# bacpop/sparrowhawk

Hardware: AMD Instinct MI355X
Metric: Gbases/s assembled, k=31 150bp reads (higher is better)
Workload: dtype u64

## Files before the change

sparrowhawk_amd/csrc/count_part.h:

```cpp
#pragma once
#include <hip/hip_runtime.h>
#include <stdint.h>
#include <type_traits>
#include "kmer.h"

namespace shk {

static constexpr int PART_THREADS = 1024;
static constexpr int COUNT_THREADS = 1024;
static constexpr int PART_MAX_P = 16384;

struct PartParams {
    uint32_t P, G, slice_cap;
    int k, m;
    uint32_t max_n;
};

template <int RW> struct Rec { uint64_t w[RW]; };

__device__ __forceinline__ uint64_t sel4(uint32_t b, uint64_t t0, uint64_t t1, uint64_t t2, uint64_t t3) {
    uint64_t lo = (b & 1) ? t1 : t0;
    uint64_t hi = (b & 1) ? t3 : t2;
    return (b & 2) ? hi : lo;
}
// ... 586 lines not shown
    const unsigned long long gbase = ((unsigned long long)ctl.emit_base_hi << 32) | ctl.emit_base_lo;
    for (uint32_t i = threadIdx.x; i < n_emit; i += COUNT_THREADS) {
        const uint32_t sl = list[i];
        const unsigned long long o = gbase + i;
        if (o < out_cap) {
            Kmer<W> x;
            if constexpr (W == 1) x.w[0] = tb.key0[sl];
            else {
#pragma unroll
                for (int j = 0; j < W; j++) x.w[j] = tb.key[j][sl];
            }
            out_keys.store(o, x);
            out_cnt[o] = tb.cnt[sl];
        }
    }
}

struct OvfRec { uint32_t p, est_distinct; unsigned long long instances; };
struct OvfItem { uint32_t p, F, cap, pad; unsigned long long base; };
static constexpr uint32_t OVF_MAX_F = 256;

struct RunView {
    const unsigned long long *run_addr16;
    const uint32_t *run_cnt;
    uint32_t S;
    int k;
    const uint32_t *weights = nullptr;
    unsigned long long rec_base16 = 0;
};

__global__ __launch_bounds__(256) void k_make_runs(const uint32_t *__restrict__ fill, PartParams pp,
                                                   const uint64_t *recs, uint32_t rec_words,
                                                   unsigned long long *__restrict__ run_addr16,
                                                   uint32_t *__restrict__ run_cnt) {
    const uint64_t n = (uint64_t)pp.P * pp.G;
    const unsigned long long base16 = (unsigned long long)recs >> 4;
    for (uint64_t i = (uint64_t)blockIdx.x * blockDim.x + threadIdx.x; i < n; i += (uint64_t)gridDim.x * blockDim.x) {
        run_addr16[i] = base16 + i * pp.slice_cap * (rec_words / 2u);
        run_cnt[i] = min(fill[i], pp.slice_cap);
    }
}

__global__ __launch_bounds__(256) void k_part_totals(const uint32_t *__restrict__ fill, PartParams pp,
                                                     unsigned long long *__restrict__ totals) {
    const uint32_t p = blockIdx.x;
    unsigned long long t = 0;
    for (uint32_t g = threadIdx.x; g < pp.G; g += blockDim.x) t += min(fill[(uint64_t)p * pp.G + g], pp.slice_cap);
    for (int o = 32; o > 0; o >>= 1) t += __shfl_down(t, o);
    __shared__ unsigned long long part[4];
    if ((threadIdx.x & 63) == 0) part[threadIdx.x >> 6] = t;
    __syncthreads();
    if (threadIdx.x == 0) totals[p] = part[0] + part[1] + part[2] + part[3];
}

template <int RW>
__global__ __launch_bounds__(256) void k_pack_partition(const uint64_t *__restrict__ recs,
                                                        const uint32_t *__restrict__ fill, PartParams pp,
                                                        const unsigned long long *__restrict__ base,
                                                        uint64_t *__restrict__ dst) {
    __shared__ uint32_t pre[257];
    const uint32_t p = blockIdx.x;
    const int lane = threadIdx.x & 63;
    if (threadIdx.x < 64) {
        uint32_t run = 0;
        for (uint32_t g0 = 0; g0 < pp.G; g0 += 64) {
            const uint32_t g = g0 + threadIdx.x;
            const uint32_t f = g < pp.G ? min(fill[(uint64_t)p * pp.G + g], pp.slice_cap) : 0u;
            uint32_t incl = f;
            for (int o = 1; o < 64; o <<= 1) { uint32_t v = __shfl_up(incl, o); if (lane >= o) incl += v; }
            if (g < pp.G) pre[g] = run + incl - f;
            run += __shfl(incl, 63);
        }
        if (threadIdx.x == 0) pre[pp.G] = run;
// ... 912 lines not shown
```

sparrowhawk_amd/csrc/pipeline.hip:

```cpp
#include <hip/hip_runtime.h>
#include <hipcub/hipcub.hpp>
#include <thread>
#include <stdint.h>
#include <stdio.h>
#include <stdlib.h>
#include <string.h>
#include <algorithm>
#include <atomic>
#include <chrono>
#include <map>
#include <memory>
#include <mutex>
#include <string>
#include <vector>

#include "kmer.h"
#include "pipeline.h"
#include "shard_comm.h"
#include "unitig_graph.h"

namespace shk {

#define HIPCHK(call)                                                                      \
    do {                                                                                  \
// ... 300 lines not shown
}

static constexpr uint32_t ARRIVAL_SLAB = 64u << 10;
__global__ __launch_bounds__(256) void k_text_to_host(const char *__restrict__ src, char *__restrict__ dst_host, unsigned long long bytes,
                                                      uint32_t n_slabs, uint32_t *__restrict__ flags_host) {
    for (uint32_t s = blockIdx.x; s < n_slabs; s += gridDim.x) {
        const unsigned long long o = (unsigned long long)s * ARRIVAL_SLAB;
        const uint32_t m = (uint32_t)(bytes - o < ARRIVAL_SLAB ? bytes - o : ARRIVAL_SLAB);
        const uint4 *a = reinterpret_cast<const uint4 *>(src + o);
        uint4 *d = reinterpret_cast<uint4 *>(dst_host + o);
        const uint32_t nv = m >> 4;
#pragma unroll 4
        for (uint32_t i = threadIdx.x; i < nv; i += 256) d[i] = a[i];
        if (threadIdx.x < (m & 15u)) dst_host[o + (nv << 4) + threadIdx.x] = src[o + (nv << 4) + threadIdx.x];
        __threadfence_system();
        __syncthreads();
        if (threadIdx.x == 0) __hip_atomic_store(&flags_host[s], 1u, __ATOMIC_RELEASE, __HIP_MEMORY_SCOPE_SYSTEM);
    }
}
__global__ __launch_bounds__(1024) void k_ends_to_host(const char *__restrict__ text, const unsigned long long *__restrict__ src ,
                                                       uint32_t nc, uint32_t E, char *__restrict__ ends_host, uint32_t *__restrict__ flag_host) {
    const unsigned long long total = (unsigned long long)nc * 2ull * E;
    for (unsigned long long t = threadIdx.x; t < total; t += blockDim.x) {
        const uint32_t c = (uint32_t)(t / (2ull * E)), r = (uint32_t)(t % (2ull * E)), side = r / E, j = r % E;
        const unsigned long long off = src[2 * c], len = src[2 * c + 1];
        const unsigned long long m = len < E ? len : (unsigned long long)E;
        char ch = 0;
        if (j < m) ch = side ? text[off + len - m + j] : text[off + j];
        ends_host[t] = ch;
    }
    __threadfence_system();
    __syncthreads();
    if (threadIdx.x == 0) __hip_atomic_store(flag_host, 1u, __ATOMIC_RELEASE, __HIP_MEMORY_SCOPE_SYSTEM);
}
__global__ __launch_bounds__(256) void k_text_to_host_planned(const char *__restrict__ src, char *__restrict__ dst_host,
                                                              const unsigned long long *__restrict__ plan) {
    if (plan[0] != 1ull) return;
    const unsigned long long bytes = plan[1];
    const unsigned long long nv = bytes >> 4;
    const uint4 *a = reinterpret_cast<const uint4 *>(src);
    uint4 *d = reinterpret_cast<uint4 *>(dst_host);
    for (unsigned long long i = (unsigned long long)blockIdx.x * 256u + threadIdx.x; i < nv; i += (unsigned long long)gridDim.x * 256u) d[i] = a[i];
    if (blockIdx.x == 0 && threadIdx.x < (bytes & 15ull)) dst_host[(nv << 4) + threadIdx.x] = src[(nv << 4) + threadIdx.x];
}
class SlabArrival : public TextArrival {
public:
    void set(char *dst, size_t bytes, volatile uint32_t *flags, uint32_t n_slabs, hipStream_t st) { base_ = dst; total_ = bytes; flags_ = flags; n_slabs_ = n_slabs; st_ = st; failed_.store(false); }
    const char *base() const override { return base_; }
    size_t total() const override { return total_; }
    static bool spin_until(volatile uint32_t *f, std::atomic<bool> &failed) {
        if (__atomic_load_n(f, __ATOMIC_ACQUIRE)) return true;
        const auto t0 = std::chrono::steady_clock::now();
        for (uint32_t it = 0;; it++) {
            if (__atomic_load_n(f, __ATOMIC_ACQUIRE)) return true;
            if (failed.load(std::memory_order_relaxed)) return false;
            if ((it & 0xFFFu) == 0xFFFu && std::chrono::steady_clock::now() - t0 > std::chrono::seconds(20)) { failed.store(true); return false; }
            __builtin_ia32_pause();
        }
    }
    void wait_range(size_t begin, size_t end) override {
        if (end > total_) end = total_;
        if (begin >= end) return;
        for (size_t s = begin / ARRIVAL_SLAB; s <= (end - 1) / ARRIVAL_SLAB; s++) if (!spin_until(flags_ + s, failed_)) return;
    }
    int finish(std::string &err) override {
        const hipError_t e = hipStreamSynchronize(st_);
        if (e != hipSuccess || failed_.load()) { err = std::string("download of the contigs failed") + (e != hipSuccess ? std::string(": ") + hipGetErrorString(e) : std::string()); return -5; }
        return 0;
    }
    std::atomic<bool> failed_{false};
private:
    char *base_ = nullptr; size_t total_ = 0; volatile uint32_t *flags_ = nullptr; uint32_t n_slabs_ = 0; hipStream_t st_ = nullptr;
};

static inline int part_win(int k) {
    static const int forced = [] { const char *e = getenv("SHK_PART_WIN"); return e ? atoi(e) : 0; }();
// ... 163 lines not shown
            if (env_u64("SHK_SLICE_NOSKEW", 0) == 0)
                while ((cap * RW * 8) % 2048 < 256 || (cap * RW * 8) % 2048 > 1792) cap++;
            if (cap * pp_.G > 0xFFFFFFF0ull) { err = "a partition would hold more than 2^32 records"; return -1; }
            pp_.slice_cap = (uint32_t)cap;
            const uint64_t n_slices = (uint64_t)P * pp_.G;
            if (int rc = recs_.alloc(n_slices * cap * RW, err)) return rc;
            if (int rc = fill_.alloc(n_slices, err)) return rc;
            HIPCHK(fill2_async(fill_.p, n_slices * 4, 0u, ctl_.p, CTL_WORDS * sizeof(unsigned long long), 0u, stream_));
            EvTimer t(stream_);
            if (h_bases && attempt == 0) {
                uint64_t C = env_u64("SHK_H2D_PIECES", 4);
                if (C < 1) C = 1;
                while (C > 1 && n_seg / C < (uint64_t)PART_THREADS * pp_.G) C--;
                if (!copy_stream_) copy_stream_ = stream_pool_get(stream_dev_ + 1000);
                if (!copy_stream_) HIPCHK(hipStreamCreateWithFlags(&copy_stream_, hipStreamNonBlocking));
                const uint64_t n_words = (n_bases + 15) / 16 + 1;
                std::vector<hipEvent_t> evs((size_t)C, nullptr);
                struct EvGuard { std::vector<hipEvent_t> &v; ~EvGuard() { for (auto e : v) if (e) (void)hipEventDestroy(e); } } evg{evs};
                struct CopyDrain { hipStream_t s; std::unique_lock<std::mutex> token; ~CopyDrain() { (void)hipStreamSynchronize(s); } }
                    copy_drain{copy_stream_, std::unique_lock<std::mutex>(upload_token(stream_dev_))};
                for (uint64_t c = 0; c < C; c++) {
                    const uint64_t s0 = n_seg * c / C, s1 = n_seg * (c + 1) / C;
                    const uint64_t w0 = h_seg_off[s0] >> 4, w1 = std::min<uint64_t>(n_words, (((uint64_t)h_seg_off[s1] + 15) >> 4) + 1);
                    HIPCHK(hipMemcpyAsync((void *)(d_seg_off + s0), h_seg_off + s0, (s1 - s0 + 1) * 4, hipMemcpyHostToDevice, copy_stream_));
                    HIPCHK(hipMemcpyAsync((void *)(d_bases + w0), h_bases + w0, (w1 - w0) * 4, hipMemcpyHostToDevice, copy_stream_));
                    HIPCHK(hipEventCreateWithFlags(&evs[c], hipEventDisableTiming));
                    HIPCHK(hipEventRecord(evs[c], copy_stream_));
                    HIPCHK(hipStreamWaitEvent(stream_, evs[c], 0));
                    launch_partition(wblk, d_bases, d_seg_off + s0, (uint32_t)(s1 - s0));
                }
                HIPCHK(hipGetLastError());
                times_.add("h2d_pieces_x1", (double)C);
                if (defer_p1_ && batches_.empty()) {
                    HIPCHK(hipMemcpyAsync(mbox64() + MB_P1, ctl_.p + 8, 16, hipMemcpyDeviceToHost, stream_));
                    t.stop_later("partition_with_upload", pending_timers_);
                    p1_ = P1Pending{true, d_bases, d_seg_off, n_seg, n_bases, cap};
                    return finish_partition(n_slices, err);
                }
                t.mark();
                unsigned long long h[2];
                HIPCHK(hipMemcpyAsync(h, ctl_.p + 8, sizeof h, hipMemcpyDeviceToHost, stream_));
                WAIT_STREAM();
                const uint32_t *fl = (const uint32_t *)&h[0];
                if (fl[1]) { err = "a read segment exceeds 32768 bases (split it on the host)"; return -1; }
                if ((uint32_t)h[1] <= cap) {
                    times_.add("partition_with_upload", t.elapsed());
                    if (int rc = finish_partition(n_slices, err)) return rc;
                    return 0;
                }
                times_.add("partition_retry", t.elapsed());
                cap = (uint64_t)(uint32_t)h[1] + 8;
                continue;
            }
            launch_partition_all(wblk, d_bases, d_seg_off, n_seg);
            HIPCHK(hipGetLastError());
            if (defer_p1_ && attempt == 0 && batches_.empty() && piece_list_.empty()) {
                HIPCHK(hipMemcpyAsync(mbox64() + MB_P1, ctl_.p + 8, 16, hipMemcpyDeviceToHost, stream_));
                t.stop_later("partition_kernel", pending_timers_);
                p1_ = P1Pending{true, d_bases, d_seg_off, n_seg, n_bases, cap};
                return finish_partition(n_slices, err);
            }
            t.mark();
            unsigned long long h[2];
            HIPCHK(hipMemcpyAsync(h, ctl_.p + 8, sizeof h, hipMemcpyDeviceToHost, stream_));
            WAIT_STREAM();
            const double ms = t.elapsed();
            const uint32_t *fl = (const uint32_t *)&h[0];
            if (fl[1]) { err = "a read segment exceeds 32768 bases (split it on the host)"; return -1; }
            const uint32_t max_fill = (uint32_t)h[1];
            if (max_fill <= cap) {
                times_.add("partition_kernel", ms);
                if (int rc = finish_partition(n_slices, err)) return rc;
                return 0;
            }
            times_.add("partition_retry", ms);
            cap = (uint64_t)max_fill + 8;
        }
        err = "partition slices overflowed twice";
        return -6;
    }

    int finish_partition(uint64_t n_slices, std::string &err) {
        constexpr int RW = 2 * W;
        have_parts_ = true;
        if (int rc = run_off_.alloc(n_slices, err)) return rc;
        if (int rc = run_cnt_.alloc(n_slices, err)) return rc;
        hipLaunchKernelGGL(k_make_runs, dim3(grid_for(n_slices)), dim3(256), 0, stream_, fill_.p, pp_, recs_.p,
                           (uint32_t)RW, run_off_.p, run_cnt_.p);
        HIPCHK(hipGetLastError());
        run_view_.run_addr16 = run_off_.p; run_view_.run_cnt = run_cnt_.p;
        run_view_.S = pp_.G; run_view_.k = k_; n_count_parts_ = pp_.P;
        return 0;
    }

    struct BatchRecs { DevBuf<uint64_t> dense; std::vector<unsigned long long> part_off;  };

    int pack_current_batch(std::string &err) {
        constexpr int RW = 2 * W;
        DevBuf<unsigned long long> tot, base;
        if (int rc = tot.alloc(pp_.P, err)) return rc;
        if (int rc = base.alloc(pp_.P, err)) return rc;
        hipLaunchKernelGGL(k_part_totals, dim3(pp_.P), dim3(256), 0, stream_, fill_.p, pp_, tot.p);
        HIPCHK(hipGetLastError());
        std::vector<unsigned long long> h(pp_.P);
        HIPCHK(hipMemcpyAsync(h.data(), tot.p, (size_t)pp_.P * 8, hipMemcpyDeviceToHost, stream_));
        WAIT_STREAM();
        std::unique_ptr<BatchRecs> b(new BatchRecs());
        b->part_off.assign(pp_.P + 1, 0);
        for (uint32_t p = 0; p < pp_.P; p++) b->part_off[p + 1] = b->part_off[p] + h[p];
        if (int rc = b->dense.alloc(b->part_off[pp_.P] * RW + 2, err)) return rc;
        HIPCHK(hipMemcpyAsync(base.p, b->part_off.data(), (size_t)pp_.P * 8, hipMemcpyHostToDevice, stream_));
        EvTimer t(stream_, stage_timers_);
        hipLaunchKernelGGL((k_pack_partition<2 * W>), dim3(pp_.P), dim3(256), 0, stream_, recs_.p, fill_.p, pp_, base.p, b->dense.p);
        HIPCHK(hipGetLastError());
        if (t.on()) times_.add("batch_pack_kernel", t.stop());
        WAIT_STREAM();
        batches_.push_back(std::move(b));
        recs_.release(); fill_.release(); run_off_.release(); run_cnt_.release(); have_parts_ = false;
        if (batches_.size() >= env_u64("SHK_MERGE_BATCHES_AT", 192)) return merge_batches(err);
        return 0;
    }

    int merge_batches(std::string &err) {
        constexpr int RW = 2 * W;
        if (batches_.size() < 2) return 0;
        if (int rc = make_batch_run_view(err)) return rc;
        std::unique_ptr<BatchRecs> m(new BatchRecs());
        m->part_off.assign(pp_.P + 1, 0);
        for (uint32_t p = 0; p < pp_.P; p++) {
            unsigned long long tot = 0;
            for (auto &b : batches_) tot += b->part_off[p + 1] - b->part_off[p];
// ... 23 lines not shown
            unsigned long long r = 0;
            for (uint32_t b = 0; b < nb; b++) r += batches_[b]->part_off[p + 1] - batches_[b]->part_off[p];
            if (r > 0xFFFFFFF0ull) { err = "a partition holds more than 2^32 records"; return -1; }
        }
        for (uint32_t p = 0; p < pp_.P; p++)
            for (uint32_t b = 0; b < nb; b++) {
                const BatchRecs &B = *batches_[b];
                const unsigned long long c = B.part_off[p + 1] - B.part_off[p];
                if (c > 0xFFFFFFFFull) { err = "partition too large in one batch"; return -1; }
                addr16[(uint64_t)p * nb + b] = ((unsigned long long)(uintptr_t)B.dense.p >> 4) + B.part_off[p] * (unsigned long long)W;
                cnt[(uint64_t)p * nb + b] = (uint32_t)c;
            }
        if (int rc = run_off_.alloc(n_runs, err)) return rc;
        if (int rc = run_cnt_.alloc(n_runs, err)) return rc;
        HIPCHK(hipMemcpyAsync(run_off_.p, addr16.data(), n_runs * 8, hipMemcpyHostToDevice, stream_));
        HIPCHK(hipMemcpyAsync(run_cnt_.p, cnt.data(), n_runs * 4, hipMemcpyHostToDevice, stream_));
        WAIT_STREAM();
        run_view_.run_addr16 = run_off_.p; run_view_.run_cnt = run_cnt_.p;
        run_view_.S = nb; run_view_.k = k_; n_count_parts_ = pp_.P;
        have_parts_ = true;
        return 0;
    }
    void set_bloom(bool on) override { bloom_ = on; }
    void set_verbose(bool on) override { if (on) { stage_timers_ = true; keep_stages_ = true; } }
    void single_batch_resident(bool on) override { defer_p1_ = on && !global_mode_; }
    void expect_more_batches() override { if (!forced_P_ && batches_.empty() && !have_parts_) forced_P_ = (uint32_t)PART_MAX_P; }

    int run_count_partitions(const RunView &rv, uint32_t n_parts, uint32_t threshold, DevBuf<uint64_t> (&keys)[W],
                             DevBuf<uint32_t> &cnt, uint64_t &n_rows, uint64_t hist_out[500], uint64_t &inst_out,
                             uint64_t cap_hint, double &ms_out, std::string &err) {
        if (n_parts == 0) { n_rows = 0; inst_out = 0; memset(hist_out, 0, 500 * 8); ms_out = 0; return 0; }
        constexpr uint32_t S = CountShared<W>::S;
        const bool repartition = env_u64("SHK_NO_REPARTITION", 0) == 0 && rv.weights == nullptr;
        DevBuf<unsigned long long> dh;
        DevBuf<OvfRec> d_ovf; DevBuf<OvfItem> d_items; DevBuf<uint32_t> d_fill, d_list, d_maxfill, d_new; DevBuf<uint64_t> d_kmers; DevBuf<BucketRef> d_blist; DevBuf<unsigned long long> d_sumfill;
        const bool bloom = bloom_ && !bloom_off_once_;
        unsigned long long bloom_new = 0, bloom_kmer_bytes = 0, bloom_kmer_bytes_exact = 0;
        if (int rc = dh.alloc(500, err)) return rc;
        if (repartition) if (int rc = d_ovf.alloc(n_parts, err)) return rc;
        const bool split = W <= 2 && repartition && !bloom && rv.weights == nullptr && split_ready_ && split_base_.size() == n_parts && split_total_ > 0 &&
                           env_u64("SHK_COUNT_SPLIT", 1) != 0;
        struct DropSplit { Pipeline<W> *me; bool on; ~DropSplit() { if (on) me->shard_drop_dedup(); } } drop_split{this, split};
        uint64_t cap = cap_hint;
        for (int attempt = 0; attempt < (bloom ? 4 : 2); attempt++) {
            bloom_new = 0; bloom_kmer_bytes = 0; bloom_kmer_bytes_exact = 0;
            for (int j = 0; j < W; j++) if (int rc = keys[j].alloc(cap, err)) return rc;
            if (int rc = cnt.alloc(cap, err)) return rc;
            HIPCHK(fill2_async(dh.p, 500 * 8, 0u, ctl_.p, CTL_WORDS * sizeof(unsigned long long), 0u, stream_));
            KeyArr<W> ok; for (int j = 0; j < W; j++) ok.w[j] = keys[j].p;
            const uint32_t probe_parts = (uint32_t)env_u64("SHK_PROBE_PARTS", 512);
            const uint32_t n_probe = (repartition && probe_parts && n_parts / 4 >= probe_parts) ? probe_parts : 0u;
            EvTimer t(stream_);
            if (split) {
                if (int rc = dd_base_.alloc(n_parts, err)) return rc;
                if (int rc = dd_n_.alloc(n_parts, err)) return rc;
                if (int rc = dd_recs_.alloc(split_total_ * 2 * W + 2, err)) return rc;
                if (int rc = dd_w_.alloc(split_total_ + 2, err)) return rc;
                if (split_stride_) {
                    hipLaunchKernelGGL(k_stride_fill, dim3((n_parts + 255) / 256), dim3(256), 0, stream_, dd_base_.p, n_parts, split_stride_);
                    HIPCHK(hipGetLastError());
                } else HIPCHK(hipMemcpyAsync(dd_base_.p, split_base_.data(), (size_t)n_parts * 8, hipMemcpyHostToDevice, stream_));
                const uint32_t defer_after = n_probe / 8;
                EvTimer t_a(stream_, stage_timers_);
                hipLaunchKernelGGL(k_dedupe_partitions<W>, dim3(std::min<uint32_t>(n_parts, 2u * (uint32_t)n_cus_)), dim3(COUNT_THREADS), 0, stream_,
                                   rv, 0u, n_parts, dd_base_.p, dd_recs_.p, dd_w_.p, dd_n_.p, (uint32_t *)(ctl_.p + 12),
                                   d_ovf.p, (uint32_t *)(ctl_.p + 3), defer_after, (S / 10) * 9, (uint32_t *)(ctl_.p + 14) + 1);
                HIPCHK(hipGetLastError());
                if (attempt == 0) t_a.stop_later("count_dedupe_kernel", pending_timers_);
                const uint32_t per_cu = 2u;
                uint32_t merge = (uint32_t)std::min<uint64_t>(std::max<uint64_t>(env_u64("SHK_COUNT_MERGE", 1), 1), 4);
                if (merge == 3) merge = 2;
                while (merge > 1 && (n_parts % merge != 0 || (n_parts / merge) % 256u != 0 || n_parts / merge < 2u * per_cu * (uint32_t)n_cus_)) merge >>= 1;
                const uint32_t n_groups = (n_parts + merge - 1) / merge;
                EmitRanges er{};
                er_groups_ = 0;
                if (n_parts % merge == 0 && (n_groups & (n_groups - 1u)) == 0 && n_groups <= GP_MAX && cap < (1ull << 28) &&
                    env_u64("SHK_GRAPH_RANGES", 1) != 0) {
                    if (int rc = er_off_.alloc(n_groups, err)) return rc;
                    if (int rc = er_msk_.alloc(n_groups, err)) return rc;
                    if (int rc = er_start_.alloc(n_groups, err)) return rc;
                    if (int rc = er_cnt_.alloc(n_groups, err)) return rc;
                    er.tab_cursor = ctl_.p + CTL_ER; er.broken = (uint32_t *)(ctl_.p + CTL_ER + 1);
                    er.off = er_off_.p; er.msk = er_msk_.p; er.start = er_start_.p; er.cnt = er_cnt_.p;
                    er_groups_ = n_groups;
                }
                hipLaunchKernelGGL(k_count_weighted<W>, dim3(std::min<uint32_t>(n_groups, per_cu * (uint32_t)n_cus_)), dim3(COUNT_THREADS), 0, stream_,
                                   dd_recs_.p, dd_w_.p, dd_base_.p, dd_n_.p, 0u, n_parts, merge, rv.k, threshold, dh.p, ok, cnt.p, (unsigned long long)cap,
                                   ctl_.p + 0, ctl_.p + 1, d_ovf.p, (uint32_t *)(ctl_.p + 3), ctl_.p + 14, 0u, defer_after, er);
            } else {
                auto kern = rv.weights ? k_count_partitions<W, true> : k_count_partitions<W, false>;
                hipLaunchKernelGGL(kern, dim3(std::min<uint32_t>(n_parts, (uint32_t)n_cus_)), dim3(COUNT_THREADS), 0, stream_, rv, n_parts, threshold,
                                   dh.p, ok, cnt.p, (unsigned long long)cap, ctl_.p + 0, ctl_.p + 1,
                                   (uint32_t *)(ctl_.p + 2), (const uint32_t *)nullptr, repartition ? d_ovf.p : (OvfRec *)nullptr,
                                   (uint32_t *)(ctl_.p + 3), (uint32_t *)(ctl_.p + 11), n_probe / 2, n_probe / 8);
            }
            HIPCHK(hipGetLastError());
            t.mark();
            unsigned long long h[4], her[2] = {0, 0};
            HIPCHK(hipMemcpyAsync(h, ctl_.p, sizeof h, hipMemcpyDeviceToHost, stream_));
            HIPCHK(hipMemcpyAsync(hist_out, dh.p, 500 * 8, hipMemcpyDeviceToHost, stream_));
            if (split && er_groups_) HIPCHK(hipMemcpyAsync(her, ctl_.p + CTL_ER, sizeof her, hipMemcpyDeviceToHost, stream_));
            WAIT_STREAM();
            ms_out = t.elapsed();
            const uint32_t n_ovf = (uint32_t)h[3];
            if (env_u64("SHK_VERBOSE_TALLY", 0)) fprintf(stderr, "[shk] pass 2: %u partitions, %u handed over, tally tried %u / over %u, split %d\n", n_parts, n_ovf,
                                                    (unsigned)((h[3] >> 32) & 0xFFFFu), (unsigned)(h[3] >> 48), (int)split);
            rows_scattered_ = (uint64_t)n_ovf * 4u > n_parts;
            if (n_ovf) {
                EvTimer t2(stream_);
                std::vector<OvfRec> ov(n_ovf);
                HIPCHK(hipMemcpy(ov.data(), d_ovf.p, (size_t)n_ovf * sizeof(OvfRec), hipMemcpyDeviceToHost));
                std::vector<OvfItem> items;
                items.reserve(n_ovf);
                std::vector<uint32_t> bad;
                uint32_t n_untried = 0;
                const unsigned long long fill_pct = env_u64("SHK_OVF_FILL_PCT", 110), cap_pct = env_u64("SHK_OVF_CAP_PCT", bloom ? 100 : 150);
                for (uint32_t i = 0; i < n_ovf; i++) {
                    if (ov[i].instances >= 0xFFFFFFF0ull) { bad.push_back(ov[i].p); continue; }
                    items.emplace_back();
                    OvfItem &item = items.back();
                    const unsigned long long per = (unsigned long long)S * fill_pct / 100;
                    const uint32_t F = (uint32_t)std::min<unsigned long long>(std::max<unsigned long long>((ov[i].instances + per - 1) / per, 2ull), OVF_MAX_F);
                    if (ov[i].est_distinct == 0) n_untried++;
                    const unsigned long long capb = ov[i].instances * cap_pct / (100ull * F) + 256;
                    item.p = ov[i].p; item.F = F; item.cap = (uint32_t)std::min<unsigned long long>(capb, 0xFFFFFFF0ull);
                    item.pad = 0; item.base = 0;
                }
                size_t n_good_total = 0;
                const int max_passes = (int)env_u64("SHK_OVF_MAX_PASSES", 4);
                for (int pass = 0; pass < max_passes && !items.empty(); pass++) {
                    const uint32_t ni = (uint32_t)items.size();
                    unsigned long long tot = 0;
                    for (auto &it : items) { it.base = tot; tot += (unsigned long long)it.F * it.cap; }
                    if (int rc = d_items.alloc(ni, err)) return rc;
                    if (int rc = d_fill.alloc((size_t)ni * OVF_MAX_F, err)) return rc;
                    if (int rc = d_kmers.alloc(tot * W, err)) return rc;
                    HIPCHK(hipMemcpyAsync(d_items.p, items.data(), (size_t)ni * sizeof(OvfItem), hipMemcpyHostToDevice, stream_));
                    if (bloom) {
                        if (int rc = d_new.alloc(ni, err)) return rc;
                        hipLaunchKernelGGL((k_ovf_scatter<W, true>), dim3(ni), dim3(COUNT_THREADS), 0, stream_, rv, d_items.p, d_kmers.p, d_fill.p, d_new.p);
                    } else {
// ... 81 lines not shown
            cap = bloom ? n_rows + n_rows / 16 + 4096 : n_rows;
        }
        err = "row buffer overflowed twice";
        return -6;
    }

    int histogram(uint64_t histo[500], uint32_t emit_threshold, std::string &err) override {
        er_ok_ = false;
        if (!global_mode_) {
            memset(histo, 0, 500 * 8);
            n_distinct_ = 0; n_emitted_ = 0; emit_threshold_ = emit_threshold;
            if (!batches_.empty()) {
                if (have_parts_ && recs_.p) if (int rc = pack_current_batch(err)) return rc;
                if (int rc = make_batch_run_view(err)) return rc;
            }
            if (have_parts_) {
                const uint64_t inst_ub_rows = total_rows_hint();
                double ms = 0; uint64_t inst = 0;
                split_base_.assign(n_count_parts_, 0); split_total_ = 0; split_stride_ = 0;
                if (batches_.empty()) {
                    split_stride_ = (unsigned long long)pp_.G * pp_.slice_cap;
                    for (uint32_t p = 0; p < n_count_parts_; p++) split_base_[p] = (unsigned long long)p * pp_.G * pp_.slice_cap;
                    split_total_ = (unsigned long long)n_count_parts_ * pp_.G * pp_.slice_cap;
                } else {
                    for (uint32_t p = 0; p < n_count_parts_; p++) {
                        split_base_[p] = split_total_;
                        for (auto &b : batches_) split_total_ += b->part_off[p + 1] - b->part_off[p];
                    }
                }
                split_ready_ = true;
                int rc_p2 = run_count_partitions(run_view_, n_count_parts_, emit_threshold, ekeys_, ecnt_, n_emitted_, histo, inst,
                                                 inst_ub_rows, ms, err);
                if (p1_.on) {
                    if (rc_p2) { std::string e2; (void)e2; (void)hipStreamSynchronize(stream_); }
                    p1_.on = false;
                    const unsigned long long *h = mbox64() + MB_P1;
                    const uint32_t *fl = (const uint32_t *)&h[0];
                    if (fl[1]) { split_ready_ = false; err = "a read segment exceeds 32768 bases (split it on the host)"; return -1; }
                    if ((uint32_t)h[1] > p1_.cap) {
                        times_.add("partition_retry", 1.0);
                        cap_override_ = (uint64_t)(uint32_t)h[1] + 8;
                        have_parts_ = false; split_ready_ = false;
                        const bool d = defer_p1_; defer_p1_ = false;
                        const int rc1 = count_batch_impl(p1_.d_bases, p1_.d_seg_off, nullptr, nullptr, p1_.n_seg, p1_.n_bases, err);
                        defer_p1_ = d;
                        if (rc1) return rc1;
                        return histogram(histo, emit_threshold, err);
                    }
                }
                if (rc_p2) { split_ready_ = false; return rc_p2; }
                split_ready_ = false;
                times_.add("count_kernel", ms);
                total_instances_ = inst;
            }
            for (int i = 0; i < 500; i++) { histo_[i] = histo[i]; n_distinct_ += histo[i]; }
            return 0;
        }
        DevBuf<unsigned long long> dh;
        if (int rc = dh.alloc(500, err)) return rc;
        HIPCHK(hipMemsetAsync(dh.p, 0, 500 * 8, stream_));
        if (tslots_) {
            EvTimer t(stream_, stage_timers_);
            hipLaunchKernelGGL(k_histogram<W>, dim3(grid_for(tslots_)), dim3(256), 0, stream_, table_view(),
                               tslots_, dh.p);
            HIPCHK(hipGetLastError());
            if (t.on()) times_.add("histogram_kernel", t.stop());
// ... 480 lines not shown
            tips_removed_ += n1; bubbles_removed_ += n2; rounds_++;
        }
        if (rounds_ > 1) if (t.on()) times_.add("correct_total", t.stop());
        corr_.release();
        return 0;
    }

    int get_adjacency(uint8_t *adj_initial, uint8_t *adj_final, uint8_t *alive, uint64_t cap,
                      std::string &err) override {
        if (!graph_ready_) { err = "graph not built"; return -2; }
        if (cap < n_solid_) { err = "buffer too small"; return -1; }
        if (!n_solid_) return 0;
        if (adj_initial && !keep_stages_) { err = "the initial adjacency is kept for inspection only on a verbose handle (or with SHK_KEEP_STAGES=1)"; return -2; }
        if (adj_initial) HIPCHK(hipMemcpy(adj_initial, adj0_.p, n_solid_, hipMemcpyDeviceToHost));
        if (adj_final) HIPCHK(hipMemcpy(adj_final, adj_.p, n_solid_, hipMemcpyDeviceToHost));
        if (alive) HIPCHK(hipMemcpy(alive, alive_.p, n_solid_, hipMemcpyDeviceToHost));
        return 0;
    }

    struct ChainState {
        DevBuf<uint32_t> spl, slot_of;
        DevBuf<uint2> winfo, ol;
        DevBuf<SegRec> segs;
        DevBuf<FragRec> frag;
        DevBuf<RankRec> Ra, Rb;
        DevBuf<FinRec> fin;
        DevBuf<HeadRec> d_heads;
        DevBuf<RingMin> ringmin;
        std::vector<HeadRec> heads;
        uint32_t seg_cap = 0;
        unsigned int n_heads = 0;
        bool heads_on_host = true;
    };
    struct EmitPlan { EmitRec *d_off; char *d_out; char *h_out; uint32_t max_heads; unsigned long long out_cap; bool planned; unsigned long long out_bytes; uint32_t n_emit; };
    int rank_chains(ChainState &cs, bool rings, std::string &err, uint32_t keep_on_device_from = 0xFFFFFFFFu, EmitPlan *plan = nullptr) {
        const uint32_t n = (uint32_t)n_solid_;
        const uint32_t total = 2 * n;
        Graph<W> g = graph_view();
        if (plan) plan->planned = false;
        const bool stage_log = getenv("SHK_STAGE_LOG") != nullptr;
        auto stage = [&](const char *what) {
            if (!stage_log) return;
            const hipError_t e = hipStreamSynchronize(stream_);
            fprintf(stderr, "[rank_chains n=%u] %s done%s\n", n, what, e == hipSuccess ? "" : " (stream error)"); fflush(stderr);
        };
        if (int rc = cs.winfo.alloc(total, err)) return rc;
        if (int rc = cs.frag.alloc(total, err)) return rc;
        if (int rc = cs.spl.alloc(total, err)) return rc;
        if (int rc = cs.ol.alloc(total, err)) return rc;
        const uint32_t split_mask = (1u << (uint32_t)env_u64("SHK_SPLIT_LOG", SPLIT_LOG_DEFAULT)) - 1u;
        const uint32_t tile_rows = (uint32_t)std::min<uint64_t>(std::max<uint64_t>(env_u64("SHK_TILE_ROWS", LF_ROWS), 1), LF_TILE / 2u);
        const int lf_grid = (int)((n + tile_rows - 1) / tile_rows);
        const uint64_t cap_all = std::min<uint64_t>((uint64_t)total + 1024u, 0xFFFFFFF0ull);
        uint64_t seg_cap64 = std::min<uint64_t>(cap_all, env_u64("SHK_SEG_CAP", (uint64_t)total / 12u + 65536u));
        constexpr unsigned int HEADS_SPEC = 512;
        static_assert(MB_MISC * 8 + HEADS_SPEC * sizeof(HeadRec) <= MBOX_BYTES, "mailbox");
        std::vector<HeadRec> &heads = cs.heads;
        unsigned long long hc[4] = {0, 0, 0, 0};
        uint32_t seg_cap = 0;
        EvTimer tr(stream_, stage_timers_);
        for (int attempt = 0;; attempt++) {
            if (attempt > 3) { err = "collapse: the chain ranking did not settle"; return -6; }
            seg_cap = (uint32_t)seg_cap64;
            cs.seg_cap = seg_cap;
            if (int rc = cs.segs.alloc(seg_cap, err)) return rc;
            if (int rc = cs.Ra.alloc(seg_cap, err)) return rc;
            if (int rc = cs.Rb.alloc(seg_cap, err)) return rc;
// ... 15 lines not shown
                               cs.spl.p, (const unsigned int *)d_nspl, cs.frag.p, cs.segs.p, split_mask, ctl_.p + 10, total, d_flags);
            stage("k_walk_frags");
            hipLaunchKernelGGL(k_orphan_cycles<W>, dim3(grid_for(total)), dim3(256), 0, stream_, g, alive_.p, cs.winfo.p, cs.ol.p,
                               cs.frag.p, cs.spl.p, cs.segs.p, d_nspl, seg_cap, d_flags, ctl_.p + 9, ctl_.p + 10);
            HIPCHK(hipGetLastError());
            stage("k_orphan_cycles");
            const int gr = grid_for((uint64_t)total / 64u + 65536u);
            int rounds = 1; { uint64_t reach = RANK_HOPS; while (reach < (uint64_t)seg_cap + 1u) { reach *= RANK_HOPS; rounds++; } }
            hipLaunchKernelGGL(k_rank_init, dim3(gr), dim3(256), 0, stream_, cs.segs.p, (const unsigned int *)d_nspl, cs.Ra.p);
            RankRec *Ri = cs.Ra.p, *Ro = cs.Rb.p;
            for (int r = 0; r < rounds; r++) {
                hipLaunchKernelGGL(k_rank_jump, dim3(gr), dim3(256), 0, stream_, (const unsigned int *)d_nspl, Ri, Ro, (uint32_t)r);
                std::swap(Ri, Ro);
            }
            stage("k_rank_jump");
            const unsigned int *d_ncyc = (const unsigned int *)(ctl_.p + 7);
            hipLaunchKernelGGL(k_rank_tails<W>, dim3(gr), dim3(256), 0, stream_, g, cs.segs.p, (const unsigned int *)d_nspl, Ri, cs.d_heads.p, cs.slot_of.p, cs.ringmin.p,
                               (unsigned int *)(ctl_.p + 6), (unsigned int *)(ctl_.p + 7));
            hipLaunchKernelGGL(k_rank_fin, dim3(gr), dim3(256), 0, stream_, cs.segs.p, (const unsigned int *)d_nspl, Ri, cs.slot_of.p, cs.fin.p);
            stage("k_rank_tails + k_rank_fin");
            hipLaunchKernelGGL(k_tile_final, dim3(lf_grid), dim3(LF_THREADS), 0, stream_, n, row_starts_.p, tile_rows, cs.ol.p, cs.frag.p, cs.fin.p, skip, (const uint32_t *)d_flags);
            stage("k_tile_final");
            if (rings) {
                hipLaunchKernelGGL(k_ring_min1<W>, dim3(1024), dim3(256), 0, stream_, g, alive_.p, cs.ol.p, cs.ringmin.p, d_ncyc);
                hipLaunchKernelGGL(k_ring_min2<W>, dim3(1024), dim3(256), 0, stream_, g, alive_.p, cs.ol.p, cs.ringmin.p, d_ncyc);
                hipLaunchKernelGGL(k_ring_rot<W>, dim3(gr), dim3(256), 0, stream_, g, cs.d_heads.p, (const unsigned int *)(ctl_.p + 6), cs.ringmin.p,
                                   cs.winfo.p, cs.ol.p, d_ncyc, d_flags);
            }
            if (plan) {
                HIPCHK(fill2_async(ctl_.p + 18, 3 * 8, 0u, nullptr, 0, 0u, stream_));
                hipLaunchKernelGGL(k_plan_emit, dim3(1), dim3(1024), 0, stream_, cs.d_heads.p, (const unsigned int *)(ctl_.p + 6), (uint32_t)k_, plan->max_heads,
                                   plan->out_cap, (const uint32_t *)d_flags, plan->d_off, ctl_.p + 18);
                hipLaunchKernelGGL(k_emit<W>, dim3(grid_for(n)), dim3(256), 0, stream_, g, alive_.p, cs.ol.p, plan->d_off, plan->d_out, (const unsigned long long *)(ctl_.p + 18));
                hipLaunchKernelGGL(k_text_to_host_planned, dim3(64), dim3(256), 0, stream_, plan->d_out, plan->h_out, (const unsigned long long *)(ctl_.p + 18));
            }
            HIPCHK(hipGetLastError());
            heads.assign(HEADS_SPEC, HeadRec());
            HIPCHK(hipMemcpyAsync(mbox64() + MB_CTL, ctl_.p, CTL_WORDS * 8, hipMemcpyDeviceToHost, stream_));
            HIPCHK(hipMemcpyAsync(mbox64() + MB_MISC, cs.d_heads.p, (size_t)std::min<uint32_t>(HEADS_SPEC, seg_cap) * sizeof(HeadRec), hipMemcpyDeviceToHost, stream_));
            WAIT_STREAM();
            const unsigned long long *hc0 = mbox64() + MB_CTL;
            if (int rc = check_graph_flags(err)) return rc;
            if (corr_pending_) {
                const unsigned int r1 = (unsigned int)hc0[16], r2 = (unsigned int)hc0[17];
                if (int rc = finish_correction(r1, r2, err)) return rc;
                if (r1 + r2 != 0) continue;
            }
            memcpy(hc, hc0 + 5, sizeof hc);
            const uint32_t flag = (uint32_t)hc[3];
            if ((flag == 4 || flag == 2) && seg_cap64 < cap_all) {
                times_.add("collapse_seg_cap_retry_x1", 1.0);
                seg_cap64 = cap_all;
                continue;
            }
            memcpy(heads.data(), mbox64() + MB_MISC, (size_t)std::min<uint32_t>(HEADS_SPEC, seg_cap) * sizeof(HeadRec));
            if (plan && hc0[18] == 1ull) { plan->planned = true; plan->out_bytes = hc0[19]; plan->n_emit = (uint32_t)hc0[20]; }
            break;
        }
        if ((uint32_t)hc[3]) { err = (uint32_t)hc[3] == 2 ? "collapse: too many short circular unitigs" : ((uint32_t)hc[3] == 3 ? "collapse: ring without a smallest k-mer" : "collapse: broken cycle"); return -6; }
        times_.add("collapse_n_splitters_x1e-3", (double)(unsigned int)hc[0] * 1e-3);
        times_.add("collapse_cycle_splitters_x1e-3", (double)(unsigned int)hc[2] * 1e-3);
        const unsigned int n_heads = (unsigned int)hc[1];
        if (tr.on()) times_.add("collapse_rank_device", tr.stop());
        cs.n_heads = n_heads;
        if (!rings || n_heads >= keep_on_device_from) { heads.resize(std::min<unsigned int>(n_heads, HEADS_SPEC)); cs.heads_on_host = false; return 0; }
        heads.resize(n_heads);
        cs.heads_on_host = true;
        if (n_heads > HEADS_SPEC)
            HIPCHK(hipMemcpy(heads.data() + HEADS_SPEC, cs.d_heads.p + HEADS_SPEC, (size_t)(n_heads - HEADS_SPEC) * sizeof(HeadRec), hipMemcpyDeviceToHost));
        return 0;
    }

    int collapse(std::vector<RawContig> &out, std::string &err, const char **json, size_t *json_len, uint64_t *n_contigs, TextArrival **arrival) override {
        out.clear();
        if (json) *json = nullptr;
        if (arrival) *arrival = nullptr;
        if (!graph_ready_) { err = "graph not built"; return -2; }
        const uint32_t n = (uint32_t)n_solid_;
        if (n == 0) return 0;
        Graph<W> g = graph_view();
        ChainState cs;
        const uint64_t dw_min = env_u64("SHK_DEVICE_WRITER_MIN", 20000);
        constexpr uint32_t PLAN_HEADS = 512;
        EmitPlan plan{}; EmitPlan *use_plan = nullptr;
        DevBuf<EmitRec> d_plan_off; DevBuf<char> d_plan_out;
        if (env_u64("SHK_DEVICE_PLAN", 0) != 0 && dw_min > PLAN_HEADS) {
            const unsigned long long cap = (unsigned long long)n + (unsigned long long)PLAN_HEADS * (unsigned long long)(k_ - 1) + 64ull;
            if (int rc = d_plan_off.alloc(PLAN_HEADS, err)) return rc;
            if (int rc = d_plan_out.alloc(cap + 16, err)) return rc;
            if (int rc = hout_.alloc(cap + 16, err)) return rc;
            plan.d_off = d_plan_off.p; plan.d_out = d_plan_out.p; plan.h_out = hout_.p; plan.max_heads = PLAN_HEADS; plan.out_cap = cap;
            use_plan = &plan;
        }
        if (int rc = rank_chains(cs, true, err, json ? (uint32_t)std::min<uint64_t>(2 * dw_min, 0xFFFFFFFFull) : 0xFFFFFFFFu, use_plan)) return rc;
        if (use_plan && plan.planned && cs.heads_on_host) {
            std::vector<HeadRec> &hd = cs.heads;
            unsigned long long at = 0; uint32_t ne = 0;
            out.reserve(plan.n_emit);
            for (size_t i = 0; i < hd.size(); i++) {
                if (!hd[i].emit) continue;
                RawContig rc; rc.kc = hd[i].kc;
                rc.ext = hout_.p + at; rc.ext_n = hd[i].len + (uint64_t)(k_ - 1);
                at += rc.ext_n; ne++;
                out.push_back(std::move(rc));
            }
            if (at != plan.out_bytes || ne != plan.n_emit) { err = "collapse: the device's emission plan and the chain records disagree"; return -6; }
            times_.add("collapse_planned_on_device_x1", 1.0);
            return 0;
        }
        if (!cs.heads_on_host) {
            const uint32_t nh = cs.n_heads;
            DevBuf<unsigned long long> sz, fl, off, idx; DevBuf<char> tmp; DevBuf<EmitRec> d_off2; DevBuf<WContig> d_c; DevBuf<char> d_out2;
            if (int rc = sz.alloc((size_t)nh + 1, err)) return rc;
            if (int rc = fl.alloc((size_t)nh + 1, err)) return rc;
            hipLaunchKernelGGL(k_w_plan_sizes, dim3(grid_for(nh)), dim3(256), 0, stream_, cs.d_heads.p, nh, (uint32_t)k_, sz.p, fl.p);
            HIPCHK(hipGetLastError());
            if (int rc = scan_excl(sz, off, nh, tmp, err)) return rc;
            if (int rc = scan_excl(fl, idx, nh, tmp, err)) return rc;
            unsigned long long last[4] = {0, 0, 0, 0};
            HIPCHK(hipMemcpyAsync(&last[0], sz.p + (nh - 1), 8, hipMemcpyDeviceToHost, stream_));
            HIPCHK(hipMemcpyAsync(&last[1], off.p + (nh - 1), 8, hipMemcpyDeviceToHost, stream_));
            HIPCHK(hipMemcpyAsync(&last[2], fl.p + (nh - 1), 8, hipMemcpyDeviceToHost, stream_));
            HIPCHK(hipMemcpyAsync(&last[3], idx.p + (nh - 1), 8, hipMemcpyDeviceToHost, stream_));
            WAIT_STREAM();
            const uint64_t out_bytes2 = last[0] + last[1], n_emit = last[2] + last[3];
            if (n_emit >= 0x7FFFFFF0ull) { err = "device writer: too many contigs"; return -1; }
            if (int rc = d_off2.alloc(nh, err)) return rc;
            if (int rc = d_c.alloc(n_emit + 1, err)) return rc;
            if (int rc = d_out2.alloc(out_bytes2 + 16, err)) return rc;
            HIPCHK(fill2_async(ctl_.p + 14, 8, 0u, nullptr, 0, 0u, stream_));
            hipLaunchKernelGGL(k_w_plan_fill, dim3(grid_for(nh)), dim3(256), 0, stream_, cs.d_heads.p, nh, (uint32_t)k_, off.p, idx.p, d_off2.p, d_c.p, (uint32_t *)(ctl_.p + 14));
            EvTimer t3(stream_, stage_timers_);
            hipLaunchKernelGGL(k_emit<W>, dim3(grid_for(n)), dim3(256), 0, stream_, g, alive_.p, cs.ol.p, d_off2.p, d_out2.p);
            HIPCHK(hipGetLastError());
            unsigned int fl9 = 0;
            if (int rc = read_ctl(fl9, 14, err)) return rc;
            if (t3.on()) times_.add("collapse_emit", t3.stop());
            if (fl9) { err = "device writer: a contig beyond 2^32 bases"; return -1; }
            if (n_emit == 0) { if (json) *json = nullptr; return 0; }
// ... 605 lines not shown
        for (size_t i = 0; i < res.contigs.size(); i++) {
            RawContig rcg; rcg.kc = res.contigs[i].kc;
            rcg.ext = hout_.p + c_off[i]; rcg.ext_n = res.contigs[i].len_nodes + (uint64_t)(k_ - 1);
            out.push_back(std::move(rcg));
        }
        times_.add("shard_assemble_host_clock", now_ms_() - t_all0);
        return 0;
    }
    template <typename F> static void host_par_ranges(size_t n, F &&fn) {
        const unsigned hw = std::thread::hardware_concurrency();
        const unsigned T = n < 262144 ? 1u : std::min(16u, std::max(1u, hw));
        if (T == 1) { fn((size_t)0, n); return; }
        std::vector<std::thread> ts;
        for (unsigned t = 1; t < T; t++) ts.emplace_back([&fn, n, t, T] { fn(n * t / T, n * (t + 1) / T); });
        fn((size_t)0, n / T);
        for (auto &t : ts) t.join();
    }
    static double now_ms_() { return std::chrono::duration<double, std::milli>(std::chrono::steady_clock::now().time_since_epoch()).count(); }

private:
    int k_;
    hipStream_t stream_ = nullptr; int stream_dev_ = 0;
    hipStream_t copy_stream_ = nullptr;
    ShardComm *wd_comm_ = nullptr;
    bool sh_agreed_ = false;
    StageTimes times_;
    std::vector<EvTimer::Pending> pending_timers_;
    int n_cus_ = 256;
    DevBuf<unsigned long long> ctl_;
    PinnedBuf mbox_;
    unsigned long long *mbox64() { return (unsigned long long *)mbox_.p; }
    static constexpr size_t MBOX_BYTES = 32768;
    static constexpr int MB_P1 = 0 , MB_CTL = 8 , MB_MISC = 64;
    struct P1Pending { bool on; const uint32_t *d_bases, *d_seg_off; uint64_t n_seg, n_bases, cap; };
    P1Pending p1_{false, nullptr, nullptr, 0, 0, 0};
    uint64_t n_host_waits_ = 0;
    bool stage_timers_ = env_u64("SHK_STAGE_TIMERS", 0) != 0;
    bool keep_stages_ = env_u64("SHK_KEEP_STAGES", 0) != 0;
    bool graph_check_pending_ = false, corr_pending_ = false, corr_tips_ = false, corr_bubbles_ = false;
    CorrScratch corr_;
    bool defer_p1_ = false;
    uint64_t cap_override_ = 0;
    DevBuf<uint64_t> tkeys_[W]; DevBuf<uint32_t> tcnt_, tstate_; uint64_t tslots_ = 0;
    struct Batch { const uint32_t *bases, *seg_off; uint64_t n_seg; };
    std::vector<Batch> pending_;
    std::vector<DevPiece> piece_list_;
    uint64_t total_instances_ = 0, n_distinct_ = 0, n_solid_ = 0;
    uint64_t histo_[500] = {0};
    bool global_mode_ = env_u64("SHK_COUNT_MODE_GLOBAL", 0) != 0;
    bool bloom_ = false, bloom_off_once_ = false;
    bool have_parts_ = false;
    bool have_dedup_ = false;
    bool split_ready_ = false;
    std::vector<unsigned long long> split_base_; unsigned long long split_total_ = 0, split_stride_ = 0;
    DevBuf<uint64_t> dd_recs_; DevBuf<uint32_t> dd_w_, dd_n_; DevBuf<unsigned long long> dd_base_;
    PartParams pp_{};
    DevBuf<uint64_t> recs_; DevBuf<uint32_t> fill_;
    DevBuf<unsigned long long> run_off_; DevBuf<uint32_t> run_cnt_;
    RunView run_view_{}; uint32_t n_count_parts_ = 0; uint32_t forced_P_ = 0;
    std::vector<std::unique_ptr<BatchRecs>> batches_;
    const void *shard_recv_ = nullptr;
    DevBuf<uint64_t> ekeys_[W]; DevBuf<uint32_t> ecnt_;
    uint64_t n_emitted_ = 0; uint32_t emit_threshold_ = 0;
    bool rows_scattered_ = false;
    DevBuf<unsigned long long> er_off_; DevBuf<uint32_t> er_msk_, er_start_, er_cnt_;
    uint32_t er_groups_ = 0; uint64_t er_rows_ = 0; bool er_ok_ = false;
    DevBuf<uint64_t> skeys_[W]; DevBuf<uint32_t> scnt_;
    DevBuf<uint64_t> gt_; DevBuf<uint8_t> gt_occ_; DevBuf<uint2> gt_scan_; uint64_t gt_slots_ = 0; uint32_t gp_ = 64;
// ... 147 lines not shown
```

Before: 177.6.

## Fold histogram zeroing into make_runs, defer P1 flag copy, enable device emit plan

Zeroing of the pass-2 histogram buffer moves into the k_make_runs kernel, and that buffer is kept as a member so pass 2 can skip its own allocation and memset. The pass-1 overflow-flag device-to-host copy is deferred so it rides along with pass-2's readback instead of being a separate transfer. The device emission plan is now on by default. Its contigs come back with one bounded hipMemcpyAsync of the planned byte count that overlaps host record building, replacing a copy kernel that wrote to pinned host memory. The aim is to cut small launches, memsets and transfers. The cost is extra state flags that must stay consistent across retry paths.

```diff
diff --git a/sparrowhawk_amd/csrc/count_part.h b/sparrowhawk_amd/csrc/count_part.h
--- a/sparrowhawk_amd/csrc/count_part.h
+++ b/sparrowhawk_amd/csrc/count_part.h
@@ -642,13 +642,16 @@
 __global__ __launch_bounds__(256) void k_make_runs(const uint32_t *__restrict__ fill, PartParams pp,
                                                    const uint64_t *recs, uint32_t rec_words,
                                                    unsigned long long *__restrict__ run_addr16,
-                                                   uint32_t *__restrict__ run_cnt) {
+                                                   uint32_t *__restrict__ run_cnt,
+                                                   unsigned long long *__restrict__ zero, uint32_t n_zero) {
     const uint64_t n = (uint64_t)pp.P * pp.G;
     const unsigned long long base16 = (unsigned long long)recs >> 4;
     for (uint64_t i = (uint64_t)blockIdx.x * blockDim.x + threadIdx.x; i < n; i += (uint64_t)gridDim.x * blockDim.x) {
         run_addr16[i] = base16 + i * pp.slice_cap * (rec_words / 2u);
         run_cnt[i] = min(fill[i], pp.slice_cap);
     }
+    if (zero)
+        for (uint32_t i = blockIdx.x * blockDim.x + threadIdx.x; i < n_zero; i += gridDim.x * blockDim.x) zero[i] = 0ull;
 }
 
 __global__ __launch_bounds__(256) void k_part_totals(const uint32_t *__restrict__ fill, PartParams pp,
diff --git a/sparrowhawk_amd/csrc/pipeline.hip b/sparrowhawk_amd/csrc/pipeline.hip
--- a/sparrowhawk_amd/csrc/pipeline.hip
+++ b/sparrowhawk_amd/csrc/pipeline.hip
@@ -356,16 +356,6 @@
     __threadfence_system();
     __syncthreads();
     if (threadIdx.x == 0) __hip_atomic_store(flag_host, 1u, __ATOMIC_RELEASE, __HIP_MEMORY_SCOPE_SYSTEM);
-}
-__global__ __launch_bounds__(256) void k_text_to_host_planned(const char *__restrict__ src, char *__restrict__ dst_host,
-                                                              const unsigned long long *__restrict__ plan) {
-    if (plan[0] != 1ull) return;
-    const unsigned long long bytes = plan[1];
-    const unsigned long long nv = bytes >> 4;
-    const uint4 *a = reinterpret_cast<const uint4 *>(src);
-    uint4 *d = reinterpret_cast<uint4 *>(dst_host);
-    for (unsigned long long i = (unsigned long long)blockIdx.x * 256u + threadIdx.x; i < nv; i += (unsigned long long)gridDim.x * 256u) d[i] = a[i];
-    if (blockIdx.x == 0 && threadIdx.x < (bytes & 15ull)) dst_host[(nv << 4) + threadIdx.x] = src[(nv << 4) + threadIdx.x];
 }
 class SlabArrival : public TextArrival {
 public:
@@ -595,10 +585,11 @@
                 HIPCHK(hipGetLastError());
                 times_.add("h2d_pieces_x1", (double)C);
                 if (defer_p1_ && batches_.empty()) {
-                    HIPCHK(hipMemcpyAsync(mbox64() + MB_P1, ctl_.p + 8, 16, hipMemcpyDeviceToHost, stream_));
+                    const bool late = p1_flags_late();
+                    if (!late) HIPCHK(hipMemcpyAsync(mbox64() + MB_P1, ctl_.p + 8, 16, hipMemcpyDeviceToHost, stream_));
                     t.stop_later("partition_with_upload", pending_timers_);
-                    p1_ = P1Pending{true, d_bases, d_seg_off, n_seg, n_bases, cap};
-                    return finish_partition(n_slices, err);
+                    p1_ = P1Pending{true, d_bases, d_seg_off, n_seg, n_bases, cap, late, false};
+                    return finish_partition(n_slices, err, late);
                 }
                 t.mark();
                 unsigned long long h[2];
@@ -618,10 +609,11 @@
             launch_partition_all(wblk, d_bases, d_seg_off, n_seg);
             HIPCHK(hipGetLastError());
             if (defer_p1_ && attempt == 0 && batches_.empty() && piece_list_.empty()) {
-                HIPCHK(hipMemcpyAsync(mbox64() + MB_P1, ctl_.p + 8, 16, hipMemcpyDeviceToHost, stream_));
+                const bool late = p1_flags_late();
+                if (!late) HIPCHK(hipMemcpyAsync(mbox64() + MB_P1, ctl_.p + 8, 16, hipMemcpyDeviceToHost, stream_));
                 t.stop_later("partition_kernel", pending_timers_);
-                p1_ = P1Pending{true, d_bases, d_seg_off, n_seg, n_bases, cap};
-                return finish_partition(n_slices, err);
+                p1_ = P1Pending{true, d_bases, d_seg_off, n_seg, n_bases, cap, late, false};
+                return finish_partition(n_slices, err, late);
             }
             t.mark();
             unsigned long long h[2];
@@ -643,14 +635,17 @@
         return -6;
     }
 
-    int finish_partition(uint64_t n_slices, std::string &err) {
+    int finish_partition(uint64_t n_slices, std::string &err, bool p2_follows = false) {
         constexpr int RW = 2 * W;
         have_parts_ = true;
+        p2_prezeroed_ = false;
         if (int rc = run_off_.alloc(n_slices, err)) return rc;
         if (int rc = run_cnt_.alloc(n_slices, err)) return rc;
+        if (p2_follows) if (int rc = dh_.alloc(500, err)) return rc;
         hipLaunchKernelGGL(k_make_runs, dim3(grid_for(n_slices)), dim3(256), 0, stream_, fill_.p, pp_, recs_.p,
-                           (uint32_t)RW, run_off_.p, run_cnt_.p);
+                           (uint32_t)RW, run_off_.p, run_cnt_.p, p2_follows ? dh_.p : (unsigned long long *)nullptr, 500u);
         HIPCHK(hipGetLastError());
+        p2_prezeroed_ = p2_follows;
         run_view_.run_addr16 = run_off_.p; run_view_.run_cnt = run_cnt_.p;
         run_view_.S = pp_.G; run_view_.k = k_; n_count_parts_ = pp_.P;
         return 0;
@@ -660,6 +655,7 @@
 
     int pack_current_batch(std::string &err) {
         constexpr int RW = 2 * W;
+        p2_prezeroed_ = false;
         DevBuf<unsigned long long> tot, base;
         if (int rc = tot.alloc(pp_.P, err)) return rc;
         if (int rc = base.alloc(pp_.P, err)) return rc;
@@ -749,11 +745,13 @@
         if (n_parts == 0) { n_rows = 0; inst_out = 0; memset(hist_out, 0, 500 * 8); ms_out = 0; return 0; }
         constexpr uint32_t S = CountShared<W>::S;
         const bool repartition = env_u64("SHK_NO_REPARTITION", 0) == 0 && rv.weights == nullptr;
-        DevBuf<unsigned long long> dh;
+        DevBuf<unsigned long long> &dh = dh_;
+        const bool prezeroed = p2_prezeroed_ && dh_.p != nullptr;
+        p2_prezeroed_ = false;
         DevBuf<OvfRec> d_ovf; DevBuf<OvfItem> d_items; DevBuf<uint32_t> d_fill, d_list, d_maxfill, d_new; DevBuf<uint64_t> d_kmers; DevBuf<BucketRef> d_blist; DevBuf<unsigned long long> d_sumfill;
         const bool bloom = bloom_ && !bloom_off_once_;
         unsigned long long bloom_new = 0, bloom_kmer_bytes = 0, bloom_kmer_bytes_exact = 0;
-        if (int rc = dh.alloc(500, err)) return rc;
+        if (!prezeroed) if (int rc = dh.alloc(500, err)) return rc;
         if (repartition) if (int rc = d_ovf.alloc(n_parts, err)) return rc;
         const bool split = W <= 2 && repartition && !bloom && rv.weights == nullptr && split_ready_ && split_base_.size() == n_parts && split_total_ > 0 &&
                            env_u64("SHK_COUNT_SPLIT", 1) != 0;
@@ -763,7 +761,7 @@
             bloom_new = 0; bloom_kmer_bytes = 0; bloom_kmer_bytes_exact = 0;
             for (int j = 0; j < W; j++) if (int rc = keys[j].alloc(cap, err)) return rc;
             if (int rc = cnt.alloc(cap, err)) return rc;
-            HIPCHK(fill2_async(dh.p, 500 * 8, 0u, ctl_.p, CTL_WORDS * sizeof(unsigned long long), 0u, stream_));
+            if (!(prezeroed && attempt == 0)) HIPCHK(fill2_async(dh.p, 500 * 8, 0u, ctl_.p, CTL_WORDS * sizeof(unsigned long long), 0u, stream_));
             KeyArr<W> ok; for (int j = 0; j < W; j++) ok.w[j] = keys[j].p;
             const uint32_t probe_parts = (uint32_t)env_u64("SHK_PROBE_PARTS", 512);
             const uint32_t n_probe = (repartition && probe_parts && n_parts / 4 >= probe_parts) ? probe_parts : 0u;
@@ -817,6 +815,12 @@
             HIPCHK(hipMemcpyAsync(h, ctl_.p, sizeof h, hipMemcpyDeviceToHost, stream_));
             HIPCHK(hipMemcpyAsync(hist_out, dh.p, 500 * 8, hipMemcpyDeviceToHost, stream_));
             if (split && er_groups_) HIPCHK(hipMemcpyAsync(her, ctl_.p + CTL_ER, sizeof her, hipMemcpyDeviceToHost, stream_));
+            const bool p1_flags_now = p1_.on && p1_.late && !p1_.copied;
+            if (p1_flags_now) {
+                HIPCHK(hipMemcpyAsync(mbox64() + MB_P1, ctl_.p + 8, 16, hipMemcpyDeviceToHost, stream_));
+                p1_.copied = true;
+                times_.add("p1_flags_with_pass2_x1", 1.0);
+            }
             WAIT_STREAM();
             ms_out = t.elapsed();
             const uint32_t n_ovf = (uint32_t)h[3];
@@ -824,6 +828,7 @@
                                                     (unsigned)((h[3] >> 32) & 0xFFFFu), (unsigned)(h[3] >> 48), (int)split);
             rows_scattered_ = (uint64_t)n_ovf * 4u > n_parts;
             if (n_ovf) {
+                if (p1_flags_now) HIPCHK(fill2_async(ctl_.p + 8, 2 * sizeof(unsigned long long), 0u, nullptr, 0, 0u, stream_));
                 EvTimer t2(stream_);
                 std::vector<OvfRec> ov(n_ovf);
                 HIPCHK(hipMemcpy(ov.data(), d_ovf.p, (size_t)n_ovf * sizeof(OvfRec), hipMemcpyDeviceToHost));
@@ -971,6 +976,10 @@
                 int rc_p2 = run_count_partitions(run_view_, n_count_parts_, emit_threshold, ekeys_, ecnt_, n_emitted_, histo, inst,
                                                  inst_ub_rows, ms, err);
                 if (p1_.on) {
+                    if (p1_.late && !p1_.copied) {
+                        (void)hipMemcpyAsync(mbox64() + MB_P1, ctl_.p + 8, 16, hipMemcpyDeviceToHost, stream_);
+                        (void)hipStreamSynchronize(stream_);
+                    }
                     if (rc_p2) { std::string e2; (void)e2; (void)hipStreamSynchronize(stream_); }
                     p1_.on = false;
                     const unsigned long long *h = mbox64() + MB_P1;
@@ -1517,7 +1526,7 @@
         unsigned int n_heads = 0;
         bool heads_on_host = true;
     };
-    struct EmitPlan { EmitRec *d_off; char *d_out; char *h_out; uint32_t max_heads; unsigned long long out_cap; bool planned; unsigned long long out_bytes; uint32_t n_emit; };
+    struct EmitPlan { EmitRec *d_off; char *d_out; uint32_t max_heads; unsigned long long out_cap; bool planned; unsigned long long out_bytes; uint32_t n_emit; };
     int rank_chains(ChainState &cs, bool rings, std::string &err, uint32_t keep_on_device_from = 0xFFFFFFFFu, EmitPlan *plan = nullptr) {
         const uint32_t n = (uint32_t)n_solid_;
         const uint32_t total = 2 * n;
@@ -1599,7 +1608,6 @@
                 hipLaunchKernelGGL(k_plan_emit, dim3(1), dim3(1024), 0, stream_, cs.d_heads.p, (const unsigned int *)(ctl_.p + 6), (uint32_t)k_, plan->max_heads,
                                    plan->out_cap, (const uint32_t *)d_flags, plan->d_off, ctl_.p + 18);
                 hipLaunchKernelGGL(k_emit<W>, dim3(grid_for(n)), dim3(256), 0, stream_, g, alive_.p, cs.ol.p, plan->d_off, plan->d_out, (const unsigned long long *)(ctl_.p + 18));
-                hipLaunchKernelGGL(k_text_to_host_planned, dim3(64), dim3(256), 0, stream_, plan->d_out, plan->h_out, (const unsigned long long *)(ctl_.p + 18));
             }
             HIPCHK(hipGetLastError());
             heads.assign(HEADS_SPEC, HeadRec());
@@ -1651,16 +1659,19 @@
         constexpr uint32_t PLAN_HEADS = 512;
         EmitPlan plan{}; EmitPlan *use_plan = nullptr;
         DevBuf<EmitRec> d_plan_off; DevBuf<char> d_plan_out;
-        if (env_u64("SHK_DEVICE_PLAN", 0) != 0 && dw_min > PLAN_HEADS) {
+        if (env_u64("SHK_DEVICE_PLAN", 1) != 0 && dw_min > PLAN_HEADS && !(arrival && getenv("SHK_ARRIVAL_MIN") != nullptr)) {
             const unsigned long long cap = (unsigned long long)n + (unsigned long long)PLAN_HEADS * (unsigned long long)(k_ - 1) + 64ull;
             if (int rc = d_plan_off.alloc(PLAN_HEADS, err)) return rc;
             if (int rc = d_plan_out.alloc(cap + 16, err)) return rc;
             if (int rc = hout_.alloc(cap + 16, err)) return rc;
-            plan.d_off = d_plan_off.p; plan.d_out = d_plan_out.p; plan.h_out = hout_.p; plan.max_heads = PLAN_HEADS; plan.out_cap = cap;
+            plan.d_off = d_plan_off.p; plan.d_out = d_plan_out.p; plan.max_heads = PLAN_HEADS; plan.out_cap = cap;
             use_plan = &plan;
         }
         if (int rc = rank_chains(cs, true, err, json ? (uint32_t)std::min<uint64_t>(2 * dw_min, 0xFFFFFFFFull) : 0xFFFFFFFFu, use_plan)) return rc;
         if (use_plan && plan.planned && cs.heads_on_host) {
+            if (plan.out_bytes > plan.out_cap) { err = "collapse: the device's emission plan exceeds its buffer"; return -6; }
+            const auto tcp = std::chrono::steady_clock::now();
+            if (plan.out_bytes) HIPCHK(hipMemcpyAsync(hout_.p, d_plan_out.p, plan.out_bytes, hipMemcpyDeviceToHost, stream_));
             std::vector<HeadRec> &hd = cs.heads;
             unsigned long long at = 0; uint32_t ne = 0;
             out.reserve(plan.n_emit);
@@ -1671,7 +1682,9 @@
                 at += rc.ext_n; ne++;
                 out.push_back(std::move(rc));
             }
+            WAIT_STREAM();
             if (at != plan.out_bytes || ne != plan.n_emit) { err = "collapse: the device's emission plan and the chain records disagree"; return -6; }
+            times_.add("collapse_d2h_contigs_host_clock", std::chrono::duration<double, std::milli>(std::chrono::steady_clock::now() - tcp).count());
             times_.add("collapse_planned_on_device_x1", 1.0);
             return 0;
         }
@@ -2343,8 +2356,11 @@
     unsigned long long *mbox64() { return (unsigned long long *)mbox_.p; }
     static constexpr size_t MBOX_BYTES = 32768;
     static constexpr int MB_P1 = 0 , MB_CTL = 8 , MB_MISC = 64;
-    struct P1Pending { bool on; const uint32_t *d_bases, *d_seg_off; uint64_t n_seg, n_bases, cap; };
-    P1Pending p1_{false, nullptr, nullptr, 0, 0, 0};
+    struct P1Pending { bool on; const uint32_t *d_bases, *d_seg_off; uint64_t n_seg, n_bases, cap; bool late , copied; };
+    P1Pending p1_{false, nullptr, nullptr, 0, 0, 0, false, false};
+    static bool p1_flags_late() { return env_u64("SHK_P1_FLAGS_EARLY", 0) == 0; }
+    DevBuf<unsigned long long> dh_;
+    bool p2_prezeroed_ = false;
     uint64_t n_host_waits_ = 0;
     bool stage_timers_ = env_u64("SHK_STAGE_TIMERS", 0) != 0;
     bool keep_stages_ = env_u64("SHK_KEEP_STAGES", 0) != 0;
```

Measured after the change: 178.0, median of 6. No clear change (+0.2%).
